# chao1224/pytorch_distributed_nn

Measured on AMD Instinct MI355X. Metric: samples/sec (whole node) ResNet-50 DDP, higher is better.
Workload: dtype bf16; 1 GPU; model=resnet50 (ImageNet layout, 224x224, 1000 classes), global_batch=256, per_gpu_batch=256, image_size=224, parallelism=dp1, optimizer=fused SGD momentum=0.9 wd=5e-5, hipgraph=False, opt_overlap=False

## Files before the change

csrc/kernels/conv3x3.hip:

```cpp
#include "conv_direct.h"

namespace {
using namespace pg;

typedef __attribute__((ext_vector_type(8))) int c3v8i;
typedef __attribute__((ext_vector_type(4))) int c3v4i;
constexpr int C3_AMAX_PARTS = 1024;
#ifndef C3_PRE_J
#define C3_PRE_J 3
#endif
#ifndef C3_F8_PRE_J
#define C3_F8_PRE_J 2
#endif

template <int FMT>
__device__ __forceinline__ uint4 c3_to_fp8(const float* v) {
    constexpr float MX = FMT ? 57344.f : 448.f;
    int w[4];
#pragma unroll
    for (int d = 0; d < 4; ++d) {
        const float c0 = fminf(fmaxf(v[4 * d], -MX), MX), c1 = fminf(fmaxf(v[4 * d + 1], -MX), MX);
        const float c2 = fminf(fmaxf(v[4 * d + 2], -MX), MX), c3 = fminf(fmaxf(v[4 * d + 3], -MX), MX);
        int x = 0;
        if constexpr (FMT) {
// ... 362 lines not shown
        for (int i = 0; i < 4; ++i)
#pragma unroll
            for (int j = 0; j < FN; ++j) acc[i][j] = f32x4_t{0.f, 0.f, 0.f, 0.f};
#pragma unroll
        for (int tap = 0; tap < 9; ++tap) {
            const int dr = tap / 3 - 1, ds = tap % 3 - 1;
            int hp[4];
#pragma unroll
            for (int f = 0; f < 4; ++f) {
                const bool v = pv[f] && (unsigned)(py[f] + dr) < (unsigned)a.H && (unsigned)(px[f] + ds) < (unsigned)a.W;
                hp[f] = v ? hb[f] + dr * a.W + ds : zpx;
            }
            const bf16_t* B = wres + tap * 4096;
#pragma unroll
            for (int ks = 0; ks < 2; ++ks) {
                bf16x8_t af[4], bfr[FN];
                const int q = ks * 4 + (lane >> 4);
#pragma unroll
                for (int f = 0; f < 4; ++f)
                    af[f] = __builtin_bit_cast(bf16x8_t, *reinterpret_cast<const u16x8_t*>(halo + halo_off(hp[f], q)));
#pragma unroll
                for (int f = 0; f < FN; ++f) bfr[f] = frag_kmajor(B, f * 16 + (lane & 15), ks, lane);
#pragma unroll
                for (int fm = 0; fm < 4; ++fm)
#pragma unroll
                    for (int fn = 0; fn < FN; ++fn)
                        acc[fm][fn] = __builtin_amdgcn_mfma_f32_16x16x32_bf16(bfr[fn], af[fm], acc[fm][fn], 0, 0, 0);
            }
        }
        c3_epilogue<NB, EPI>(a, acc, tile, p0, 0, wave, lane, pv);
    }
}

template <int KC, int NB, int EPI, bool PRE, bool FP = false>
__global__ void __launch_bounds__(256, 2) conv1x1_areg_kernel(C3Args a) {
    constexpr int FN = NB / 16, NKS = 2 * KC, K = 64 * KC;
    constexpr int BPT = NB * KC * 8 / 256;
    static_assert(BPT >= 1 && NB * KC * 8 % 256 == 0, "weight step must cover the block");
    extern __shared__ __attribute__((aligned(16))) char smem[];
    bf16_t* const bbuf = reinterpret_cast<bf16_t*>(smem);
    const int tid = threadIdx.x, lane = tid & 63, wave = tid >> 6;
    const int groups = a.ntiles;
    const int t = xcd_remap(blockIdx.x, a.tiles * groups);
    const int tile = t / groups, grp = t - tile * groups;
    const int steps = (a.N / NB) / groups;
    const int c00 = grp * steps;
    const int p0 = tile * C3_BM;

    u16x8_t rb[BPT];
    auto load_b = [&](int s) {
        const int n0 = (c00 + s) * NB;
#pragma unroll
        for (int i = 0; i < BPT; ++i) {
            const int li = tid + 256 * i, row = li / (KC * 8), rem = li - row * (KC * 8);
            rb[i] = *reinterpret_cast<const u16x8_t*>(a.w + (long)(n0 + row) * K + rem * 8);
        }
    };
    auto store_b = [&](int buf) {
        bf16_t* B = bbuf + buf * (KC * NB * 64);
#pragma unroll
        for (int i = 0; i < BPT; ++i) {
            const int li = tid + 256 * i, row = li / (KC * 8), rem = li - row * (KC * 8);
            *reinterpret_cast<u16x8_t*>(B + (rem >> 3) * (NB * 64) + kimg_off(row, rem & 7)) = rb[i];
        }
    };
    load_b(0);

    bool pv[4];
    long prow[4];
#pragma unroll
    for (int fm = 0; fm < 4; ++fm) {
        const int p = p0 + wave * 64 + fm * 16 + (lane & 15);
        pv[fm] = p < a.P;
        prow[fm] = (long)(pv[fm] ? p : a.P - 1) * K;
    }
    bf16x8_t af[NKS][4];
    if constexpr (!PRE) {
        [[maybe_unused]] float* coef = reinterpret_cast<float*>(bbuf + 2 * KC * NB * 64);
        if constexpr (FP) {
            for (int c = tid; c < K; c += 256) {
                coef[c] = a.pro_sc[c];
                coef[K + c] = a.pro_sh[c];
            }
            __syncthreads();
        }
#pragma unroll
        for (int ks = 0; ks < NKS; ++ks)
#pragma unroll
            for (int fm = 0; fm < 4; ++fm) {
                u16x8_t v = *reinterpret_cast<const u16x8_t*>(a.x + prow[fm] + ks * 32 + (lane >> 4) * 8);
                if constexpr (FP) v = fpro_apply_lds<K>(coef, ks * 32 + (lane >> 4) * 8, v);
                af[ks][fm] = __builtin_bit_cast(bf16x8_t, v);
            }
    } else {
        float* coef = reinterpret_cast<float*>(bbuf + 2 * KC * NB * 64);
        {
            const float invL = (float)(1.0 / (double)a.P);
            for (int c = tid; c < K; c += 256) {
                const float is = a.pre_invstd[c], kk = (a.pre_gamma ? a.pre_gamma[c] : 1.f) * is;
                const float dg = a.pre_dgamma[c] * invL, db = a.pre_dbeta[c] * invL;
                coef[c] = kk;
                coef[K + c] = -kk * is * dg;
                coef[2 * K + c] = kk * (a.pre_mean[c] * is * dg - db);
            }
        }
        __syncthreads();
        constexpr int GB = KC == 4 ? 2 : (KC == 2 ? 4 : 2);
#pragma unroll
        for (int g0 = 0; g0 < NKS; g0 += GB) {
            u16x8_t v[GB][4], tv[GB][4];
#pragma unroll
            for (int kk = 0; kk < GB; ++kk)
#pragma unroll
                for (int fm = 0; fm < 4; ++fm) {
                    const long off = prow[fm] + (g0 + kk) * 32 + (lane >> 4) * 8;
                    v[kk][fm] = *reinterpret_cast<const u16x8_t*>(a.x + off);
                    tv[kk][fm] = *reinterpret_cast<const u16x8_t*>(a.pre_t + off);
                }
#pragma unroll
            for (int kk = 0; kk < GB; ++kk) {
                const int k = (g0 + kk) * 32 + (lane >> 4) * 8;
                PreCoef pc;
#pragma unroll
                for (int j = 0; j < 8; ++j) {
                    pc.k[j] = coef[k + j];
                    pc.A[j] = coef[K + k + j];
                    pc.B[j] = coef[2 * K + k + j];
                }
#pragma unroll
                for (int fm = 0; fm < 4; ++fm) {
                    const u16x8_t d = pre_apply(pc, v[kk][fm], tv[kk][fm]);
                    if (a.pre_out && grp == 0 && pv[fm]) *reinterpret_cast<u16x8_t*>(a.pre_out + prow[fm] + k) = d;
                    af[g0 + kk][fm] = __builtin_bit_cast(bf16x8_t, d);
                }
            }
        }
    }
    store_b(0);
    __syncthreads();

    for (int s = 0; s < steps; ++s) {
        const bool more = s + 1 < steps;
        if (more) load_b(s + 1);
        const bf16_t* B = bbuf + (s & 1) * (KC * NB * 64);
        f32x4_t acc[4][FN];
#pragma unroll
        for (int i = 0; i < 4; ++i)
#pragma unroll
            for (int j = 0; j < FN; ++j) acc[i][j] = f32x4_t{0.f, 0.f, 0.f, 0.f};
        bf16x8_t bcur[FN], bnxt[FN];
#pragma unroll
        for (int f = 0; f < FN; ++f) bcur[f] = frag_kmajor(B, f * 16 + (lane & 15), 0, lane);
#pragma unroll
        for (int ks = 0; ks < NKS; ++ks) {
            if (ks + 1 < NKS) {
#pragma unroll
                for (int f = 0; f < FN; ++f)
                    bnxt[f] = frag_kmajor(B + ((ks + 1) >> 1) * (NB * 64), f * 16 + (lane & 15), (ks + 1) & 1, lane);
            }
#pragma unroll
            for (int fm = 0; fm < 4; ++fm)
#pragma unroll
                for (int fn = 0; fn < FN; ++fn)
                    acc[fm][fn] = __builtin_amdgcn_mfma_f32_16x16x32_bf16(bcur[fn], af[ks][fm], acc[fm][fn], 0, 0, 0);
            __builtin_amdgcn_sched_barrier(0);
#pragma unroll
            for (int f = 0; f < FN; ++f) bcur[f] = bnxt[f];
        }
        if (more) store_b((s + 1) & 1);
        c3_epilogue<NB, EPI>(a, acc, tile, p0, (c00 + s) * NB, wave, lane, pv);
        if (more) __syncthreads();
    }
}

int c3r_smem(int W);

__global__ void __launch_bounds__(256) conv3x3_flip_kernel(const bf16_t* __restrict__ w, bf16_t* __restrict__ wt,
                                                           int K, int C) {
    const long n = 9L * K * C;
    for (long i = (long)blockIdx.x * 256 + threadIdx.x; i < n; i += (long)gridDim.x * 256) {
        const int c = (int)(i % C);
        const long r1 = i / C;
        const int tap = (int)(r1 % 9);
        const int k = (int)(r1 / 9);
        wt[((long)c * 9 + (8 - tap)) * K + k] = w[i];
    }
}

int c3_halo_max(int W) {
    const int rows = (C3_BM - 1 + W - 1) / W + 1 + 2;
    return rows * W;
}

__global__ void __launch_bounds__(256) conv3x3_flip8_kernel(const uint8_t* __restrict__ w, uint8_t* __restrict__ wt,
                                                            int K, int C) {
    const long n = 9L * K * C;
    for (long i = (long)blockIdx.x * 256 + threadIdx.x; i < n; i += (long)gridDim.x * 256) {
        const int k = (int)(i % K);
        const long r0 = i / K;
        const int tap = (int)(r0 % 9), c = (int)(r0 / 9);
        wt[i] = w[((long)k * 9 + (8 - tap)) * C + c];
    }
}
// ... 13 lines not shown
    }
    const int grid = a.tiles < grid_cus() ? a.tiles : grid_cus();
    hipLaunchKernelGGL((conv3x3_w64_kernel<EPI>), dim3(grid), dim3(256), sm, st, a);
    PDNN_LAUNCH_RET;
}

template <int NB, int EPI, bool PRE, int F8 = 0, bool FP = false>
int c3_launch(const C3Args& a, hipStream_t st) {
    static int attr_done = 0;
    const int sm = c3_smem<NB>(a.W);
    if (sm > attr_done) {
        (void)hipFuncSetAttribute((const void*)conv3x3_kernel<NB, EPI, PRE, F8, FP>,
                                  hipFuncAttributeMaxDynamicSharedMemorySize, sm);
        attr_done = sm;
    }
    hipLaunchKernelGGL((conv3x3_kernel<NB, EPI, PRE, F8, FP>), dim3(a.tiles * a.ntiles), dim3(256), sm, st, a);
    PDNN_LAUNCH_RET;
}

template <int NB, bool PRE>
int c3_dispatch(const C3Args& a, int epi, hipStream_t st) {
    switch (epi) {
        case C3_BNB: return c3_launch<NB, C3_BNB, PRE>(a, st);
        case C3_STATS: return c3_launch<NB, C3_STATS, PRE>(a, st);
        case C3_RES: return c3_launch<NB, C3_RES, PRE>(a, st);
        default: return c3_launch<NB, C3_PLAIN, PRE>(a, st);
    }
}

}



template <int KC, int NB, int EPI, bool PRE, bool FP = false>
int areg_launch(const C3Args& a, hipStream_t st) {
    constexpr int sm = 2 * KC * NB * 128 + (PRE ? 3 * 64 * KC * 4 : (FP ? 2 * 64 * KC * 4 : 0));
    hipLaunchKernelGGL((conv1x1_areg_kernel<KC, NB, EPI, PRE, FP>), dim3(a.tiles * a.ntiles), dim3(256), sm, st, a);
    PDNN_LAUNCH_RET;
}

template <int KC, int NB, bool PRE>
int areg_dispatch(const C3Args& a, int epi, hipStream_t st) {
    if constexpr (!PRE) {
        if (a.pro_sc) {
            if (epi == C3_STATS) return areg_launch<KC, NB, C3_STATS, false, true>(a, st);
            if (epi == C3_PLAIN) return areg_launch<KC, NB, C3_PLAIN, false, true>(a, st);
            return (int)hipErrorInvalidValue;
        }
    }
    switch (epi) {
        case C3_BNB: return areg_launch<KC, NB, C3_BNB, PRE>(a, st);
        case C3_STATS: return areg_launch<KC, NB, C3_STATS, PRE>(a, st);
        case C3_RES: return areg_launch<KC, NB, C3_RES, PRE>(a, st);
        default: return areg_launch<KC, NB, C3_PLAIN, PRE>(a, st);
    }
}

template <bool PRE>
int areg_run(C3Args& a, int K, int epi, hipStream_t st) {
    const int nb = K == 256 ? 32 : 64;
    const int chunks = a.N / nb;
    int g = 1;
    while (g < chunks && (long)a.tiles * g < 512 && chunks % (2 * g) == 0) g *= 2;
    a.ntiles = g;
    if (K == 64) return areg_dispatch<1, 64, PRE>(a, epi, st);
    if (K == 128) return areg_dispatch<2, 64, PRE>(a, epi, st);
    return areg_dispatch<4, 32, PRE>(a, epi, st);
}

static bool set_pre(C3Args& a, const bf16_t* t, const float* mean, const float* invstd, const float* gamma,
             const float* dgamma, const float* dbeta, bf16_t* out) {
    a.pre_t = t; a.pre_mean = mean; a.pre_invstd = invstd; a.pre_gamma = gamma;
    a.pre_dgamma = dgamma; a.pre_dbeta = dbeta; a.pre_out = out;
    if (!t) return !out;
    return mean && invstd && dgamma && dbeta;
}
static int c3_force() { return pg::tune().conv3x3_force; }

static FastDiv make_fdiv_c3(uint32_t d) {
    FastDiv f;
    f.d = d ? d : 1;
    uint32_t l = 0;
    while ((1ull << l) < f.d) ++l;
    f.s = l;
    f.m = (uint32_t)((((1ull << l) - f.d) << 32) / f.d + 1);
    return f;
}

PDNN_API int pdnn_conv3x3_supported(int Nimg, int H, int W, int C, int N) {
    if (C % 64 || N % 64 || C < 64 || N < 64 || W < 1 || H < 1) return 0;
    if (W < 12 && !c3_force()) return 0;
    if ((long)Nimg * H * W >= (1L << 31) / 2) return 0;
    const int nb = N % 128 == 0 ? 128 : 64;
    const int sm = nb == 128 ? c3_smem<128>(W) : c3_smem<64>(W);
    return sm <= 80 * 1024 ? 1 : 0;
}

PDNN_API int pdnn_conv3x3_force(int f) {
    const int old = c3_force();
    pg::tune().conv3x3_force = f ? 1 : 0;
// ... 84 lines not shown
    C3Args a{};
    a.x = x; a.w = reinterpret_cast<const bf16_t*>(wq); a.y = y;
    a.Nimg = Nimg; a.H = H; a.W = W; a.C = C; a.N = N; a.P = Nimg * H * W;
    a.dW = make_fdiv_c3(W); a.dH = make_fdiv_c3(H);
    a.tiles = (int)cdiv(a.P, C3_BM);
    a.halo_max = c3_halo_max(W);
    a.stats = stats;
    if (!set_pre(a, pre_t, pre_mean, pre_invstd, pre_gamma, pre_dgamma, pre_dbeta, pre_out))
        return (int)hipErrorInvalidValue;
    a.ep_x = bn_x; a.ep_mean = bn_mean; a.ep_invstd = bn_invstd; a.ep_mscale = bn_mscale; a.ep_mshift = bn_mshift;
    if (bn_x && !stats) return (int)hipErrorInvalidValue;
    a.f8_scale = scale; a.f8_inv = inv; a.f8_winv = winv; a.f8_amax = amax;
    a.ntiles = N / 128;
    const bool pre = pre_t != nullptr;
    if (e5m2) {
        if (bn_x) return pre ? c3_launch<128, C3_BNB, true, 2>(a, st) : c3_launch<128, C3_BNB, false, 2>(a, st);
        if (stats) return (int)hipErrorInvalidValue;
        return pre ? c3_launch<128, C3_PLAIN, true, 2>(a, st) : c3_launch<128, C3_PLAIN, false, 2>(a, st);
    }
    if (pre || bn_x) return (int)hipErrorInvalidValue;
    if (!pro_sc != !pro_sh) return (int)hipErrorInvalidValue;
    if (pro_sc) {
        a.pro_sc = pro_sc; a.pro_sh = pro_sh;
        return stats ? c3_launch<128, C3_STATS, false, 1, true>(a, st) : c3_launch<128, C3_PLAIN, false, 1, true>(a, st);
    }
    return stats ? c3_launch<128, C3_STATS, false, 1>(a, st) : c3_launch<128, C3_PLAIN, false, 1>(a, st);
}

PDNN_API int pdnn_conv1x1_panel_supported(long P, int K, int N) {
    const bool k_ok = K == 64 || K == 128 || K == 256;
    return k_ok && N % 64 == 0 && N >= 64 && P > 0 && P < (1L << 30) ? 1 : 0;
}

PDNN_API int pdnn_conv1x1_panel(const bf16_t* x, const bf16_t* w, bf16_t* y, long P, int K, int N, float* stats,
                                const bf16_t* res, const uint8_t* res_mask, const bf16_t* bn_x, const float* bn_mean,
                                const float* bn_invstd, const float* bn_mscale, const float* bn_mshift,
                                const bf16_t* pre_t, const float* pre_mean, const float* pre_invstd,
                                const float* pre_gamma, const float* pre_dgamma, const float* pre_dbeta,
                                bf16_t* pre_out, const float* pro_sc, const float* pro_sh, hipStream_t st) {
    if (!pdnn_conv1x1_panel_supported(P, K, N) || (bn_x && !stats) || (res_mask && !res) || (!pro_sc != !pro_sh) ||
        (pro_sc && (pre_t || bn_x || res)))
        return (int)hipErrorInvalidValue;
    C3Args a{};
    a.x = x; a.w = w; a.y = y; a.C = K; a.N = N; a.P = (int)P;
    a.tiles = (int)cdiv(P, C3_BM);
    a.stats = stats; a.res = res; a.rmask = res_mask;
    a.ep_x = bn_x; a.ep_mean = bn_mean; a.ep_invstd = bn_invstd; a.ep_mscale = bn_mscale; a.ep_mshift = bn_mshift;
    if (!set_pre(a, pre_t, pre_mean, pre_invstd, pre_gamma, pre_dgamma, pre_dbeta, pre_out))
        return (int)hipErrorInvalidValue;
    a.pro_sc = pro_sc; a.pro_sh = pro_sh;
    const int epi = bn_x ? C3_BNB : (stats ? C3_STATS : (res ? C3_RES : C3_PLAIN));
    return pre_t ? areg_run<true>(a, K, epi, st) : areg_run<false>(a, K, epi, st);
}

PDNN_API int pdnn_conv1x1_panel_stats_rows(long P) { return (int)cdiv(P, C3_BM) * 4; }
```

csrc/kernels/conv_direct.h:

```cpp
#pragma once
#include "gemm_common.h"
#include "tuning.h"

namespace {
using namespace pg;

constexpr int C3_BM = 256;
enum { C3_PLAIN = 0, C3_STATS = 1, C3_BNB = 2, C3_RES = 3 };

struct C3Args {
    const bf16_t* x;
    const bf16_t* w;
    bf16_t* y;
    int Nimg, H, W, C, N, P;
    FastDiv dW, dH;
    int tiles, ntiles;
    int halo_max;
    float* stats;
    const bf16_t* res;
    const uint8_t* rmask;
    const bf16_t* ep_x;
    const float *ep_mean, *ep_invstd, *ep_mscale, *ep_mshift;
    const bf16_t* pre_t;
    const float *pre_mean, *pre_invstd, *pre_gamma, *pre_dgamma, *pre_dbeta;
// ... 59 lines not shown
        coef[c] = a.pro_sc[c0 + c];
        coef[CH + c] = a.pro_sh[c0 + c];
    }
}
template <int CH>
__device__ __forceinline__ u16x8_t fpro_apply_lds(const float* coef, int c, const u16x8_t& v) {
    float x[8], sc[8], sh[8];
    unpack8(v, x);
    *reinterpret_cast<float4*>(sc) = *reinterpret_cast<const float4*>(coef + c);
    *reinterpret_cast<float4*>(sc + 4) = *reinterpret_cast<const float4*>(coef + c + 4);
    *reinterpret_cast<float4*>(sh) = *reinterpret_cast<const float4*>(coef + CH + c);
    *reinterpret_cast<float4*>(sh + 4) = *reinterpret_cast<const float4*>(coef + CH + c + 4);
#pragma unroll
    for (int j = 0; j < 8; ++j) x[j] = fmaxf(fmaf(x[j], sc[j], sh[j]), 0.f);
    return pack8(x);
}

__device__ __forceinline__ u16x8_t mask16(const u16x8_t& v, bool ok) {
    const uint32_t m = ok ? 0xFFFFFFFFu : 0u;
    uint4 u = __builtin_bit_cast(uint4, v);
    u.x &= m; u.y &= m; u.z &= m; u.w &= m;
    return __builtin_bit_cast(u16x8_t, u);
}

__device__ __forceinline__ u16x8_t c3_zero8() {
    u16x8_t z = {0, 0, 0, 0, 0, 0, 0, 0};
    return z;
}

__device__ __forceinline__ int halo_off(int hp, int q) {
    return hp * 64 + ((q ^ ((hp >> 1) & 7)) << 3);
}

template <int NB, int EPI>
struct C3PairOps {
    static constexpr bool RES = EPI == C3_RES, BNB = EPI == C3_BNB;
    u16x4_t tv[(RES || BNB) ? 2 : 1][4];
    uint32_t mw[RES ? 4 : 1];
};

template <int NB, int EPI>
__device__ __forceinline__ void c3_load_pair(const C3Args& a, const long (&lrow)[4], int n0, int lg, int fp,
                                             C3PairOps<NB, EPI>& o) {
    constexpr bool RES = EPI == C3_RES, BNB = EPI == C3_BNB;
    if constexpr (RES) {
#pragma unroll
        for (int fm = 0; fm < 4; ++fm)
            o.mw[fm] = a.rmask ? *reinterpret_cast<const uint32_t*>(a.rmask + ((lrow[fm] + n0 + 32 * fp) >> 3))
                               : 0xFFFFFFFFu;
    }
    if constexpr (RES || BNB) {
        const bf16_t* src = BNB ? a.ep_x : a.res;
#pragma unroll
        for (int h = 0; h < 2; ++h) {
            const int n = n0 + (2 * fp + h) * 16 + 4 * lg;
#pragma unroll
            for (int fm = 0; fm < 4; ++fm) o.tv[h][fm] = *reinterpret_cast<const u16x4_t*>(src + lrow[fm] + n);
        }
    }
}

template <int NB, int EPI>
__device__ __forceinline__ void c3_epilogue_rows(const C3Args& a, f32x4_t (&acc)[4][NB / 16], int tile,
                                                 const long (&orow)[4], int n0, int wave, int lane,
                                                 const bool (&pv)[4]) {
    constexpr int FN = NB / 16, NP = FN / 2;
    constexpr bool RES = EPI == C3_RES;
    const int lg = lane >> 4;
    long lrow[4];
#pragma unroll
    for (int fm = 0; fm < 4; ++fm) lrow[fm] = pv[fm] ? orow[fm] : 0;
    C3PairOps<NB, EPI> cur, nxt;
    if constexpr (NP > 1) c3_load_pair<NB, EPI>(a, lrow, n0, lg, 0, cur);
    else if constexpr (RES) {
#pragma unroll
        for (int fm = 0; fm < 4; ++fm)
            cur.mw[fm] = a.rmask ? *reinterpret_cast<const uint32_t*>(a.rmask + ((lrow[fm] + n0) >> 3)) : 0xFFFFFFFFu;
    }
#pragma unroll
    for (int fp = 0; fp < NP; ++fp) {
        if (fp + 1 < NP) c3_load_pair<NB, EPI>(a, lrow, n0, lg, fp + 1, nxt);
        uint32_t pk[4][2][2];
#pragma unroll
        for (int h = 0; h < 2; ++h) {
            const int fn = 2 * fp + h;
            const int n = n0 + fn * 16 + 4 * lg;
            float s[4] = {0, 0, 0, 0}, q[4] = {0, 0, 0, 0};
            float bms[4], bmh[4];
            if constexpr (NP == 1 && (RES || EPI == C3_BNB)) {
                const bf16_t* src = EPI == C3_BNB ? a.ep_x : a.res;
#pragma unroll
                for (int fm = 0; fm < 4; ++fm)
                    cur.tv[h][fm] = pv[fm] ? *reinterpret_cast<const u16x4_t*>(src + orow[fm] + n) : u16x4_t{0, 0, 0, 0};
            }
            if constexpr (EPI == C3_BNB) {
                const float4 m4 = *reinterpret_cast<const float4*>(a.ep_mscale + n);
                const float4 h4 = *reinterpret_cast<const float4*>(a.ep_mshift + n);
                bms[0] = m4.x; bms[1] = m4.y; bms[2] = m4.z; bms[3] = m4.w;
                bmh[0] = h4.x; bmh[1] = h4.y; bmh[2] = h4.z; bmh[3] = h4.w;
            }
#pragma unroll
            for (int fm = 0; fm < 4; ++fm) {
                const bool ok = pv[fm];
                float v[4];
#pragma unroll
                for (int j = 0; j < 4; ++j) v[j] = acc[fm][fn][j];
                if constexpr (RES) {
                    const uint32_t mb = cur.mw[fm] >> (16 * h + 4 * lg);
#pragma unroll
                    for (int j = 0; j < 4; ++j) v[j] += ((mb >> j) & 1) ? bf2f(cur.tv[h][fm][j]) : 0.f;
                }
                if constexpr (EPI == C3_BNB) {
#pragma unroll
                    for (int j = 0; j < 4; ++j) {
                        const float tt = bf2f(cur.tv[h][fm][j]);
                        const float gm = (ok && fmaf(tt, bms[j], bmh[j]) > 0.f) ? bf2f(f2bf(v[j])) : 0.f;
                        v[j] = gm;
                        s[j] += gm;
                        q[j] += gm * tt;
                    }
                } else if constexpr (EPI == C3_STATS) {
                    if (ok) {
#pragma unroll
                        for (int j = 0; j < 4; ++j) {
                            const float r = bf2f(f2bf(v[j]));
                            s[j] += r;
                            q[j] += r * r;
                        }
                    }
                }
                pk[fm][h][0] = pk2bf(v[0], v[1]);
                pk[fm][h][1] = pk2bf(v[2], v[3]);
            }
            if constexpr (EPI == C3_STATS || EPI == C3_BNB) {
#pragma unroll
                for (int j = 0; j < 4; ++j) {
                    s[j] = row16_sum(s[j]);
                    q[j] = row16_sum(q[j]);
                }
                {
                    float* ps = stat_row(a.stats, (long)tile * 4 + wave, a.N) + n;
                    if constexpr (EPI == C3_BNB) {
                        const int j = lane & 3;
                        if ((lane & 12) == 4) {
                            const float qj = (sel4(q, j) - a.ep_mean[n + j] * sel4(s, j)) * a.ep_invstd[n + j];
                            q[0] = q[1] = q[2] = q[3] = qj;
                        }
                    }
                    stat_add_frag(ps, ps + a.N, lane, s, q, true);
                }
            }
        }
#pragma unroll
        for (int fm = 0; fm < 4; ++fm) {
            const auto s0 = __builtin_amdgcn_permlane16_swap(pk[fm][0][0], pk[fm][1][0], false, false);
            const auto s1 = __builtin_amdgcn_permlane16_swap(pk[fm][0][1], pk[fm][1][1], false, false);
            const int n = n0 + (2 * fp + (lg & 1)) * 16 + 8 * (lg >> 1);
            if (pv[fm]) *reinterpret_cast<uint4*>(a.y + orow[fm] + n) = make_uint4(s0[0], s1[0], s0[1], s1[1]);
        }
        if (fp + 1 < NP) cur = nxt;
    }
}

template <int NB, int EPI>
__device__ __forceinline__ void c3_epilogue(const C3Args& a, f32x4_t (&acc)[4][NB / 16], int tile, int p0, int n0,
                                            int wave, int lane, const bool (&pv)[4]) {
    long orow[4];
#pragma unroll
    for (int fm = 0; fm < 4; ++fm) orow[fm] = (long)(p0 + wave * 64 + fm * 16 + (lane & 15)) * a.N;
    c3_epilogue_rows<NB, EPI>(a, acc, tile, orow, n0, wave, lane, pv);
}

}
```

pytorch_distributed_nn_amd/ops/_backend.py:

```python
from __future__ import annotations

import ctypes
import functools
import os
from pathlib import Path

import torch

_LIBDIR = Path(__file__).resolve().parent.parent / "_lib"
_LIB = None
_ERR = None

P = ctypes.c_void_p
I = ctypes.c_int
L = ctypes.c_long
F = ctypes.c_float
D = ctypes.c_double

_SIGS = {
    "pdnn_gemm_nt": [P, L, P, L, P, L, I, I, I, F, P, I, I, P],
    "pdnn_gemm_nn": [P, L, P, L, P, L, I, I, I, F, I, P],
    "pdnn_gemm_tn_acc": [P, L, P, L, P, L, I, I, I, F, P],
    "pdnn_conv_fwd": [P, P, P, I, I, I, I, I, I, I, I, I, I, I, P, P, P, P],
    "pdnn_conv_dgrad": [P, P, P, I, I, I, I, I, I, I, I, I, I, I, P, P, P, P, P, P, P, P, P],
    "pdnn_conv_dgrad_stats_rows": [I, I, I, I, I, I, I],
    "pdnn_conv_wgrad": [P, P, P, I, I, I, I, I, I, I, I, I, I, I, P, P, P],
    "pdnn_gemm_stats_rows": [I],
    "pdnn_conv3x3": [P, P, P, I, I, I, I, I, P, P, P, P, P, P, P, P, I, P, P, P, P, P, P, P, P, P, P],
    "pdnn_conv3x3_supported": [I, I, I, I, I],
    "pdnn_conv3x3s2": [P, P, P, I, I, I, I, I, I, P] + [P] * 5 + [P] * 7 + [P, P, I, P],
    "pdnn_conv3x3s2_supported": [I, I, I, I, I],
    "pdnn_conv3x3s2_wgrad": [P, P, P, I, I, I, I, I, P, P, P, P],
    "pdnn_conv3x3s2_wgrad_supported": [I, I, I, I, I],
    "pdnn_conv3x3s2_wgrad_ws": [I, I, I, I, I],
    "pdnn_conv3x3_fp8_supported": [I, I, I, I, I],
    "pdnn_conv3x3_stats_rows": [I, I, I],
    "pdnn_conv3x3_flip": [P, P, I, I, P],
    "pdnn_conv3x3_flip8": [P, P, I, I, P],
    "pdnn_conv3x3_fp8": [P, P, P, I, I, I, I, I, P] + [P] * 5 + [P] * 7 + [P] * 4 + [I, P, P, P],
    "pdnn_conv3x3_wgrad": [P, P, P, I, I, I, I, I, P, P, P, P],
    "pdnn_conv3x3_wgrad_fp8": [P, P, P, I, I, I, I, I, P, P, P, P, P, P, P, P],
    "pdnn_conv3x3_wgrad_supported": [I, I, I, I, I],
    "pdnn_conv3x3_wgrad_ws": [I, I, I, I, I],
    "pdnn_conv3x3_force": [I],
    "pdnn_tune_set": [ctypes.c_char_p, I],
    "pdnn_tune_get": [ctypes.c_char_p],
    "pdnn_tune_list": [ctypes.c_char_p, I],
    "pdnn_tune_error": [],
    "pdnn_tune_unknown": [],
    "pdnn_set_comm_world": [I],
    "pdnn_grid_cus": [],
    "pdnn_conv1x1_panel": [P, P, P, L, I, I, P, P, P, P, P, P, P, P, P, P, P, P, P, P, P, P, P, P],
    "pdnn_conv1x1_panel_supported": [L, I, I],
    "pdnn_conv1x1_panel_stats_rows": [L],
    "pdnn_conv1x1_wide": [P, P, P, L, I, I] + [P] * 16,
    "pdnn_conv1x1_wide_supported": [L, I, I],
    "pdnn_stem_conv": [P, P, P, I, I, I, I, I, P, P],
    "pdnn_stem_stats_rows": [L],
    "pdnn_stem_conv_nchw": [P, P, P, I, I, I, I, I, P, P],
    "pdnn_stem_wgrad_nchw": [P, P, P, I, I, I, I, I, P, P, P, P, P, P, P, P, P, P, P],
    "pdnn_stem_wgrad_ws": [I, I, I],
    "pdnn_bn_relu_maxpool": [P, P, P, P, P, I, I, I, I, I, I, P],
    "pdnn_set_glds_mode": [I],
    "pdnn_set_pp_mode": [I],
    "pdnn_set_pp_bn": [I],
    "pdnn_set_pp_trace": [P],
    "pdnn_pp_wgrad": [P, L, P, L, P, L, I, I, I, F, P, I, P, I, P],
    "pdnn_pp_wgrad_plan": [I, I, I, I],
    "pdnn_pp_wgrad_splits": [I, I, I],
    "pdnn_pp_wgrad_ws": [I, I, I],
    "pdnn_pp_wgrad_splits_long": [I, I, I],
    "pdnn_pp_gemm_nt_splitk": [P, L, P, L, P, L, I, I, I, P, I, P],
    "pdnn_pp_splitk_splits": [I, I, I],
    "pdnn_transpose_bf16": [P, L, P, L, I, I, P],
    "pdnn_subsample": [P, P, I, I, I, I, I, P],
    "pdnn_transpose_bf16_multi": [P, P, P, P, I, P],
    "pdnn_set_staged_store": [I],
    "pdnn_bn_reduce_rows": [L, I],
    "pdnn_bn_finalize": [P, I, I, D, F, F, P, P, P, P, P, P, P, P, P],
    "pdnn_bn_eval_coeff": [I, F, P, P, P, P, P, P, P],
    "pdnn_bn_stats": [P, L, I, P, P],
    "pdnn_bn_apply": [P, L, I, P, P, P, P, P, I, P, P, P],
    "pdnn_bn_bwd_reduce": [P, P, L, I, P, P, I, P, P, P, P, P, P, P, P, P],
    "pdnn_bn_bwd_finalize": [P, I, I, P, P, I, P, P, P],
    "pdnn_bn_bwd_apply": [P, P, L, I, P, P, P, P, P, I, P, P, P, P, P, P, P, P, P, P, P, P, P],
# ... 176 lines not shown
```

pytorch_distributed_nn_amd/ops/kernels.py:

```python
from __future__ import annotations

import ctypes

import torch

from ._backend import _CUR_DEV, HipError, call, lib, ptr, stream

BF16 = torch.bfloat16
F32 = torch.float32


def _chk(cond, msg):
    if not cond:
        raise ValueError(msg)


def _is_krsc(w):
    K, C, R, S = w.shape
    return w.stride() == (R * S * C, 1, S * C, C)


def _bf16_c(t, name):
    _chk(t.dtype == BF16 and t.is_cuda, f"{name}: expected CUDA bf16, got {t.dtype} {t.device}")
    _chk(t.is_contiguous(), f"{name}: expected contiguous tensor")
# ... 236 lines not shown

def _panel_ok(P, K, N, R, S, st, pad, fwd=False):
    return (_P1["mode"] and R == 1 and S == 1 and st == 1 and pad == 0
            and (lib().pdnn_conv1x1_panel_supported(P, K, N) == 1 or _wide_ok(P, K, N, fwd)))


def _pre_args(pre, x):
    if pre is None:
        return (None,) * 7
    t, mean, inv, gamma, dg, db, dt_out = pre
    _bf16_c(t, "pre.t")
    _chk(t.numel() == x.numel(), "pre: t must have the operand's shape")
    if dt_out is not None:
        _chk(dt_out.numel() == x.numel() and dt_out.dtype == BF16 and dt_out.is_contiguous(), "pre: dt_out")
    return tuple(ptr(v) for v in (t, mean, inv, gamma, dg, db, dt_out))


def conv1x1_panel(x2d, w2d, want_stats=False, res=None, bn=None, res_mask=None, out=None, pre=None, pro=None):
    P, Kc = x2d.shape
    N = w2d.shape[0]
    y = out if out is not None else torch.empty(P, N, device=x2d.device, dtype=BF16)
    slab = None
    t = mean = inv = msc = msh = None
    if want_stats or bn is not None:
        slab = stat_bins(N, x2d.device)
    if bn is not None:
        t, mean, inv, msc, msh = bn
    if Kc >= 512:
        _chk(pro is None, "conv1x1_panel: the forward prologue needs K <= 256")
        call("pdnn_conv1x1_wide", ptr(x2d), ptr(w2d), ptr(y), P, Kc, N, ptr(slab), ptr(res), ptr(res_mask), ptr(t),
             ptr(mean), ptr(inv), ptr(msc), ptr(msh), *_pre_args(pre, x2d), stream())
        return y, slab
    psc, psh = pro if pro is not None else (None, None)
    call("pdnn_conv1x1_panel", ptr(x2d), ptr(w2d), ptr(y), P, Kc, N, ptr(slab), ptr(res), ptr(res_mask), ptr(t),
         ptr(mean), ptr(inv), ptr(msc), ptr(msh), *_pre_args(pre, x2d), ptr(psc), ptr(psh), stream())
    return y, slab


def conv3x3_flip(w):
    K, R, S, C = w.shape
    wt = torch.empty(C, 3, 3, K, device=w.device, dtype=BF16)
    call("pdnn_conv3x3_flip", ptr(w), ptr(wt), K, C, stream())
    return wt


def conv3x3(x, w, want_stats=False, res=None, bn=None, out=None, res_mask=None, pre=None, pro=None):
    Nimg, H, W, C = x.shape
    Ko = w.shape[0]
    y = out if out is not None else torch.empty(Nimg, H, W, Ko, device=x.device, dtype=BF16)
    slab = None
    t = mean = inv = msc = msh = None
    if want_stats or bn is not None:
        slab = stat_bins(Ko, x.device)
    if bn is not None:
        t, mean, inv, msc, msh = bn
    psc, psh = pro if pro is not None else (None, None)
    call("pdnn_conv3x3", ptr(x), ptr(w), ptr(y), Nimg, H, W, C, Ko, ptr(slab), ptr(res), ptr(res_mask), ptr(t),
         ptr(mean), ptr(inv), ptr(msc), ptr(msh), _C3["nb"], *_pre_args(pre, x), ptr(psc), ptr(psh), stream())
    return y, slab


def conv_fwd(x, w, st, pad, pro=None, want_stats=False):
    _bf16_c(x, "conv_fwd.x")
    N, H, W, C = x.shape
    _bf16_c(w, "conv_fwd.w")
    K, R, S, C2 = w.shape
# ... 910 lines not shown
```

pytorch_distributed_nn_amd/tuning.py:

```python
from __future__ import annotations

import os

DEFAULTS = {"side_wgrad": 1, "wide1x1_dgrad": 1, "a2_fold": 1, "wt_prefetch": 0, "wt_layer_batch": 1, "colsum_atomic": 1, "bias_in_wgrad": 1, "s2_halo": 3, "ds_sub": 1, "wgrad1x1_pp_pix": 200704, "gpt2_side_wgrad": 1, "xent_fused": 1, "wgrad_plan_cus": 128}

_VALUES = dict(DEFAULTS)


def _parse(s: str) -> dict:
    out = {}
    for item in filter(None, (p.strip() for p in s.split(","))):
        if "=" not in item:
            raise ValueError(f"PDNN_TUNE: {item!r} is not key=value")
        k, v = item.split("=", 1)
        out[k.strip()] = int(v)
    return out


for _k, _v in _parse(os.environ.get("PDNN_TUNE", "")).items():
    if _k in _VALUES:
        _VALUES[_k] = _v


def get(key: str) -> int:
    return _VALUES[key]


def set(key: str, value: int) -> int:
    if key not in _VALUES:
        raise KeyError(f"unknown tuning key {key!r} (kernel-side keys: ops.kernels.tune_set)")
    old = _VALUES[key]
    _VALUES[key] = int(value)
    return old
```

Measured before the change: 12300 samples/s.

## Add half-height row tiles with higher occupancy for 1x1 panel conv kernel

Templates the 1x1 register-A panel conv kernel and its epilogue on the number of 16-row fragments per wave (4 or 2). The 2-fragment variant uses 128-row pixel tiles and a launch bound of 3 blocks per SM, and the column-group split now targets 768 slots. A heuristic picks the half tile by default for large pixel counts (P >= 50176) in the supported K=128/256 epilogue combinations, and a new tuning key can force either size. The aim is more resident waves and better latency hiding on the big ResNet 1x1 layers. In exchange each block reuses each weight step across fewer rows, weight traffic per output rises, and the register budget per thread is tighter.

```diff
diff --git a/csrc/kernels/conv3x3.hip b/csrc/kernels/conv3x3.hip
--- a/csrc/kernels/conv3x3.hip
+++ b/csrc/kernels/conv3x3.hip
@@ -418,9 +418,11 @@
     }
 }
 
-template <int KC, int NB, int EPI, bool PRE, bool FP = false>
-__global__ void __launch_bounds__(256, 2) conv1x1_areg_kernel(C3Args a) {
+template <int KC, int NB, int EPI, bool PRE, bool FP = false, int FM = 4, int WPS = 2>
+__global__ void __launch_bounds__(256, WPS) conv1x1_areg_kernel(C3Args a) {
     constexpr int FN = NB / 16, NKS = 2 * KC, K = 64 * KC;
+    constexpr int BMA = 64 * FM;
+    static_assert(FM == 4 || FM == 2, "row fragments per wave");
     constexpr int BPT = NB * KC * 8 / 256;
     static_assert(BPT >= 1 && NB * KC * 8 % 256 == 0, "weight step must cover the block");
     extern __shared__ __attribute__((aligned(16))) char smem[];
@@ -431,7 +433,7 @@
     const int tile = t / groups, grp = t - tile * groups;
     const int steps = (a.N / NB) / groups;
     const int c00 = grp * steps;
-    const int p0 = tile * C3_BM;
+    const int p0 = tile * BMA;
 
     u16x8_t rb[BPT];
     auto load_b = [&](int s) {
@@ -452,15 +454,15 @@
     };
     load_b(0);
 
-    bool pv[4];
-    long prow[4];
-#pragma unroll
-    for (int fm = 0; fm < 4; ++fm) {
-        const int p = p0 + wave * 64 + fm * 16 + (lane & 15);
+    bool pv[FM];
+    long prow[FM];
+#pragma unroll
+    for (int fm = 0; fm < FM; ++fm) {
+        const int p = p0 + wave * (16 * FM) + fm * 16 + (lane & 15);
         pv[fm] = p < a.P;
         prow[fm] = (long)(pv[fm] ? p : a.P - 1) * K;
     }
-    bf16x8_t af[NKS][4];
+    bf16x8_t af[NKS][FM];
     if constexpr (!PRE) {
         [[maybe_unused]] float* coef = reinterpret_cast<float*>(bbuf + 2 * KC * NB * 64);
         if constexpr (FP) {
@@ -473,7 +475,7 @@
 #pragma unroll
         for (int ks = 0; ks < NKS; ++ks)
 #pragma unroll
-            for (int fm = 0; fm < 4; ++fm) {
+            for (int fm = 0; fm < FM; ++fm) {
                 u16x8_t v = *reinterpret_cast<const u16x8_t*>(a.x + prow[fm] + ks * 32 + (lane >> 4) * 8);
                 if constexpr (FP) v = fpro_apply_lds<K>(coef, ks * 32 + (lane >> 4) * 8, v);
                 af[ks][fm] = __builtin_bit_cast(bf16x8_t, v);
@@ -491,14 +493,15 @@
             }
         }
         __syncthreads();
-        constexpr int GB = KC == 4 ? 2 : (KC == 2 ? 4 : 2);
+        constexpr int GB4 = KC == 4 ? 2 : (KC == 2 ? 4 : 2);
+        constexpr int GB = GB4 * (4 / FM) < NKS ? GB4 * (4 / FM) : NKS;
 #pragma unroll
         for (int g0 = 0; g0 < NKS; g0 += GB) {
-            u16x8_t v[GB][4], tv[GB][4];
+            u16x8_t v[GB][FM], tv[GB][FM];
 #pragma unroll
             for (int kk = 0; kk < GB; ++kk)
 #pragma unroll
-                for (int fm = 0; fm < 4; ++fm) {
+                for (int fm = 0; fm < FM; ++fm) {
                     const long off = prow[fm] + (g0 + kk) * 32 + (lane >> 4) * 8;
                     v[kk][fm] = *reinterpret_cast<const u16x8_t*>(a.x + off);
                     tv[kk][fm] = *reinterpret_cast<const u16x8_t*>(a.pre_t + off);
@@ -514,7 +517,7 @@
                     pc.B[j] = coef[2 * K + k + j];
                 }
 #pragma unroll
-                for (int fm = 0; fm < 4; ++fm) {
+                for (int fm = 0; fm < FM; ++fm) {
                     const u16x8_t d = pre_apply(pc, v[kk][fm], tv[kk][fm]);
                     if (a.pre_out && grp == 0 && pv[fm]) *reinterpret_cast<u16x8_t*>(a.pre_out + prow[fm] + k) = d;
                     af[g0 + kk][fm] = __builtin_bit_cast(bf16x8_t, d);
@@ -529,9 +532,9 @@
         const bool more = s + 1 < steps;
         if (more) load_b(s + 1);
         const bf16_t* B = bbuf + (s & 1) * (KC * NB * 64);
-        f32x4_t acc[4][FN];
-#pragma unroll
-        for (int i = 0; i < 4; ++i)
+        f32x4_t acc[FM][FN];
+#pragma unroll
+        for (int i = 0; i < FM; ++i)
 #pragma unroll
             for (int j = 0; j < FN; ++j) acc[i][j] = f32x4_t{0.f, 0.f, 0.f, 0.f};
         bf16x8_t bcur[FN], bnxt[FN];
@@ -545,7 +548,7 @@
                     bnxt[f] = frag_kmajor(B + ((ks + 1) >> 1) * (NB * 64), f * 16 + (lane & 15), (ks + 1) & 1, lane);
             }
 #pragma unroll
-            for (int fm = 0; fm < 4; ++fm)
+            for (int fm = 0; fm < FM; ++fm)
 #pragma unroll
                 for (int fn = 0; fn < FN; ++fn)
                     acc[fm][fn] = __builtin_amdgcn_mfma_f32_16x16x32_bf16(bcur[fn], af[ks][fm], acc[fm][fn], 0, 0, 0);
@@ -554,7 +557,7 @@
             for (int f = 0; f < FN; ++f) bcur[f] = bnxt[f];
         }
         if (more) store_b((s + 1) & 1);
-        c3_epilogue<NB, EPI>(a, acc, tile, p0, (c00 + s) * NB, wave, lane, pv);
+        c3_epilogue<NB, EPI, FM>(a, acc, tile, p0, (c00 + s) * NB, wave, lane, pv);
         if (more) __syncthreads();
     }
 }
@@ -634,40 +637,66 @@
 
 
 
-template <int KC, int NB, int EPI, bool PRE, bool FP = false>
+template <int FM>
+constexpr int areg_wps() {
+    return FM == 4 ? 2 : 3;
+}
+
+constexpr bool areg_half_has(int KC, int epi, bool pre, bool fp) {
+    return !fp && (KC == 4 ? epi != C3_STATS : (KC == 2 && epi == C3_RES && pre));
+}
+
+template <int KC, int NB, int EPI, bool PRE, bool FP = false, int FM = 4>
 int areg_launch(const C3Args& a, hipStream_t st) {
-    constexpr int sm = 2 * KC * NB * 128 + (PRE ? 3 * 64 * KC * 4 : (FP ? 2 * 64 * KC * 4 : 0));
-    hipLaunchKernelGGL((conv1x1_areg_kernel<KC, NB, EPI, PRE, FP>), dim3(a.tiles * a.ntiles), dim3(256), sm, st, a);
-    PDNN_LAUNCH_RET;
-}
-
-template <int KC, int NB, bool PRE>
+    if constexpr (FM == 2 && !areg_half_has(KC, EPI, PRE, FP)) {
+        return (int)hipErrorInvalidValue;
+    } else {
+        constexpr int sm = 2 * KC * NB * 128 + (PRE ? 3 * 64 * KC * 4 : (FP ? 2 * 64 * KC * 4 : 0));
+        hipLaunchKernelGGL((conv1x1_areg_kernel<KC, NB, EPI, PRE, FP, FM, areg_wps<FM>()>), dim3(a.tiles * a.ntiles),
+                           dim3(256), sm, st, a);
+        PDNN_LAUNCH_RET;
+    }
+}
+
+template <int KC, int NB, bool PRE, int FM>
 int areg_dispatch(const C3Args& a, int epi, hipStream_t st) {
     if constexpr (!PRE) {
         if (a.pro_sc) {
-            if (epi == C3_STATS) return areg_launch<KC, NB, C3_STATS, false, true>(a, st);
-            if (epi == C3_PLAIN) return areg_launch<KC, NB, C3_PLAIN, false, true>(a, st);
+            if (epi == C3_STATS) return areg_launch<KC, NB, C3_STATS, false, true, FM>(a, st);
+            if (epi == C3_PLAIN) return areg_launch<KC, NB, C3_PLAIN, false, true, FM>(a, st);
             return (int)hipErrorInvalidValue;
         }
     }
     switch (epi) {
-        case C3_BNB: return areg_launch<KC, NB, C3_BNB, PRE>(a, st);
-        case C3_STATS: return areg_launch<KC, NB, C3_STATS, PRE>(a, st);
-        case C3_RES: return areg_launch<KC, NB, C3_RES, PRE>(a, st);
-        default: return areg_launch<KC, NB, C3_PLAIN, PRE>(a, st);
-    }
+        case C3_BNB: return areg_launch<KC, NB, C3_BNB, PRE, false, FM>(a, st);
+        case C3_STATS: return areg_launch<KC, NB, C3_STATS, PRE, false, FM>(a, st);
+        case C3_RES: return areg_launch<KC, NB, C3_RES, PRE, false, FM>(a, st);
+        default: return areg_launch<KC, NB, C3_PLAIN, PRE, false, FM>(a, st);
+    }
+}
+
+static int areg_fm(long P, int K, int epi, bool pre, bool fp, int rows) {
+    if (rows == 4 || !areg_half_has(K / 64, epi, pre, fp)) return 4;
+    return rows == 2 || P >= 50176 ? 2 : 4;
 }
 
 template <bool PRE>
-int areg_run(C3Args& a, int K, int epi, hipStream_t st) {
+int areg_run(C3Args& a, int K, int epi, int rows, hipStream_t st) {
+    const int fm = areg_fm(a.P, K, epi, PRE, a.pro_sc != nullptr, rows);
+    a.tiles = (int)cdiv((long)a.P, 64 * fm);
     const int nb = K == 256 ? 32 : 64;
     const int chunks = a.N / nb;
+    const long slots = fm == 4 ? 512 : 768;
     int g = 1;
-    while (g < chunks && (long)a.tiles * g < 512 && chunks % (2 * g) == 0) g *= 2;
+    while (g < chunks && (long)a.tiles * g < slots && chunks % (2 * g) == 0) g *= 2;
     a.ntiles = g;
-    if (K == 64) return areg_dispatch<1, 64, PRE>(a, epi, st);
-    if (K == 128) return areg_dispatch<2, 64, PRE>(a, epi, st);
-    return areg_dispatch<4, 32, PRE>(a, epi, st);
+    if (fm == 2) {
+        if (K == 128) return areg_dispatch<2, 64, PRE, 2>(a, epi, st);
+        return areg_dispatch<4, 32, PRE, 2>(a, epi, st);
+    }
+    if (K == 64) return areg_dispatch<1, 64, PRE, 4>(a, epi, st);
+    if (K == 128) return areg_dispatch<2, 64, PRE, 4>(a, epi, st);
+    return areg_dispatch<4, 32, PRE, 4>(a, epi, st);
 }
 
 static bool set_pre(C3Args& a, const bf16_t* t, const float* mean, const float* invstd, const float* gamma,
@@ -818,25 +847,36 @@
     return k_ok && N % 64 == 0 && N >= 64 && P > 0 && P < (1L << 30) ? 1 : 0;
 }
 
+PDNN_API int pdnn_conv1x1_panel_tile(const bf16_t* x, const bf16_t* w, bf16_t* y, long P, int K, int N, float* stats,
+                                     const bf16_t* res, const uint8_t* res_mask, const bf16_t* bn_x,
+                                     const float* bn_mean, const float* bn_invstd, const float* bn_mscale,
+                                     const float* bn_mshift, const bf16_t* pre_t, const float* pre_mean,
+                                     const float* pre_invstd, const float* pre_gamma, const float* pre_dgamma,
+                                     const float* pre_dbeta, bf16_t* pre_out, const float* pro_sc, const float* pro_sh,
+                                     int rows, hipStream_t st) {
+    if (!pdnn_conv1x1_panel_supported(P, K, N) || (bn_x && !stats) || (res_mask && !res) || (!pro_sc != !pro_sh) ||
+        (pro_sc && (pre_t || bn_x || res)) || (rows != 0 && rows != 2 && rows != 4))
+        return (int)hipErrorInvalidValue;
+    C3Args a{};
+    a.x = x; a.w = w; a.y = y; a.C = K; a.N = N; a.P = (int)P;
+    a.stats = stats; a.res = res; a.rmask = res_mask;
+    a.ep_x = bn_x; a.ep_mean = bn_mean; a.ep_invstd = bn_invstd; a.ep_mscale = bn_mscale; a.ep_mshift = bn_mshift;
+    if (!set_pre(a, pre_t, pre_mean, pre_invstd, pre_gamma, pre_dgamma, pre_dbeta, pre_out))
+        return (int)hipErrorInvalidValue;
+    a.pro_sc = pro_sc; a.pro_sh = pro_sh;
+    const int epi = bn_x ? C3_BNB : (stats ? C3_STATS : (res ? C3_RES : C3_PLAIN));
+    return pre_t ? areg_run<true>(a, K, epi, rows, st) : areg_run<false>(a, K, epi, rows, st);
+}
+
 PDNN_API int pdnn_conv1x1_panel(const bf16_t* x, const bf16_t* w, bf16_t* y, long P, int K, int N, float* stats,
                                 const bf16_t* res, const uint8_t* res_mask, const bf16_t* bn_x, const float* bn_mean,
                                 const float* bn_invstd, const float* bn_mscale, const float* bn_mshift,
                                 const bf16_t* pre_t, const float* pre_mean, const float* pre_invstd,
                                 const float* pre_gamma, const float* pre_dgamma, const float* pre_dbeta,
                                 bf16_t* pre_out, const float* pro_sc, const float* pro_sh, hipStream_t st) {
-    if (!pdnn_conv1x1_panel_supported(P, K, N) || (bn_x && !stats) || (res_mask && !res) || (!pro_sc != !pro_sh) ||
-        (pro_sc && (pre_t || bn_x || res)))
-        return (int)hipErrorInvalidValue;
-    C3Args a{};
-    a.x = x; a.w = w; a.y = y; a.C = K; a.N = N; a.P = (int)P;
-    a.tiles = (int)cdiv(P, C3_BM);
-    a.stats = stats; a.res = res; a.rmask = res_mask;
-    a.ep_x = bn_x; a.ep_mean = bn_mean; a.ep_invstd = bn_invstd; a.ep_mscale = bn_mscale; a.ep_mshift = bn_mshift;
-    if (!set_pre(a, pre_t, pre_mean, pre_invstd, pre_gamma, pre_dgamma, pre_dbeta, pre_out))
-        return (int)hipErrorInvalidValue;
-    a.pro_sc = pro_sc; a.pro_sh = pro_sh;
-    const int epi = bn_x ? C3_BNB : (stats ? C3_STATS : (res ? C3_RES : C3_PLAIN));
-    return pre_t ? areg_run<true>(a, K, epi, st) : areg_run<false>(a, K, epi, st);
+    return pdnn_conv1x1_panel_tile(x, w, y, P, K, N, stats, res, res_mask, bn_x, bn_mean, bn_invstd, bn_mscale,
+                                   bn_mshift, pre_t, pre_mean, pre_invstd, pre_gamma, pre_dgamma, pre_dbeta, pre_out,
+                                   pro_sc, pro_sh, 0, st);
 }
 
 PDNN_API int pdnn_conv1x1_panel_stats_rows(long P) { return (int)cdiv(P, C3_BM) * 4; }
diff --git a/csrc/kernels/conv_direct.h b/csrc/kernels/conv_direct.h
--- a/csrc/kernels/conv_direct.h
+++ b/csrc/kernels/conv_direct.h
@@ -115,20 +115,20 @@
     return hp * 64 + ((q ^ ((hp >> 1) & 7)) << 3);
 }
 
-template <int NB, int EPI>
+template <int NB, int EPI, int FMR = 4>
 struct C3PairOps {
     static constexpr bool RES = EPI == C3_RES, BNB = EPI == C3_BNB;
-    u16x4_t tv[(RES || BNB) ? 2 : 1][4];
-    uint32_t mw[RES ? 4 : 1];
+    u16x4_t tv[(RES || BNB) ? 2 : 1][FMR];
+    uint32_t mw[RES ? FMR : 1];
 };
 
-template <int NB, int EPI>
-__device__ __forceinline__ void c3_load_pair(const C3Args& a, const long (&lrow)[4], int n0, int lg, int fp,
-                                             C3PairOps<NB, EPI>& o) {
+template <int NB, int EPI, int FMR = 4>
+__device__ __forceinline__ void c3_load_pair(const C3Args& a, const long (&lrow)[FMR], int n0, int lg, int fp,
+                                             C3PairOps<NB, EPI, FMR>& o) {
     constexpr bool RES = EPI == C3_RES, BNB = EPI == C3_BNB;
     if constexpr (RES) {
 #pragma unroll
-        for (int fm = 0; fm < 4; ++fm)
+        for (int fm = 0; fm < FMR; ++fm)
             o.mw[fm] = a.rmask ? *reinterpret_cast<const uint32_t*>(a.rmask + ((lrow[fm] + n0 + 32 * fp) >> 3))
                                : 0xFFFFFFFFu;
     }
@@ -138,32 +138,32 @@
         for (int h = 0; h < 2; ++h) {
             const int n = n0 + (2 * fp + h) * 16 + 4 * lg;
 #pragma unroll
-            for (int fm = 0; fm < 4; ++fm) o.tv[h][fm] = *reinterpret_cast<const u16x4_t*>(src + lrow[fm] + n);
+            for (int fm = 0; fm < FMR; ++fm) o.tv[h][fm] = *reinterpret_cast<const u16x4_t*>(src + lrow[fm] + n);
         }
     }
 }
 
-template <int NB, int EPI>
-__device__ __forceinline__ void c3_epilogue_rows(const C3Args& a, f32x4_t (&acc)[4][NB / 16], int tile,
-                                                 const long (&orow)[4], int n0, int wave, int lane,
-                                                 const bool (&pv)[4]) {
+template <int NB, int EPI, int FMR = 4>
+__device__ __forceinline__ void c3_epilogue_rows(const C3Args& a, f32x4_t (&acc)[FMR][NB / 16], int tile,
+                                                 const long (&orow)[FMR], int n0, int wave, int lane,
+                                                 const bool (&pv)[FMR]) {
     constexpr int FN = NB / 16, NP = FN / 2;
     constexpr bool RES = EPI == C3_RES;
     const int lg = lane >> 4;
-    long lrow[4];
-#pragma unroll
-    for (int fm = 0; fm < 4; ++fm) lrow[fm] = pv[fm] ? orow[fm] : 0;
-    C3PairOps<NB, EPI> cur, nxt;
-    if constexpr (NP > 1) c3_load_pair<NB, EPI>(a, lrow, n0, lg, 0, cur);
+    long lrow[FMR];
+#pragma unroll
+    for (int fm = 0; fm < FMR; ++fm) lrow[fm] = pv[fm] ? orow[fm] : 0;
+    C3PairOps<NB, EPI, FMR> cur, nxt;
+    if constexpr (NP > 1) c3_load_pair<NB, EPI, FMR>(a, lrow, n0, lg, 0, cur);
     else if constexpr (RES) {
 #pragma unroll
-        for (int fm = 0; fm < 4; ++fm)
+        for (int fm = 0; fm < FMR; ++fm)
             cur.mw[fm] = a.rmask ? *reinterpret_cast<const uint32_t*>(a.rmask + ((lrow[fm] + n0) >> 3)) : 0xFFFFFFFFu;
     }
 #pragma unroll
     for (int fp = 0; fp < NP; ++fp) {
-        if (fp + 1 < NP) c3_load_pair<NB, EPI>(a, lrow, n0, lg, fp + 1, nxt);
-        uint32_t pk[4][2][2];
+        if (fp + 1 < NP) c3_load_pair<NB, EPI, FMR>(a, lrow, n0, lg, fp + 1, nxt);
+        uint32_t pk[FMR][2][2];
 #pragma unroll
         for (int h = 0; h < 2; ++h) {
             const int fn = 2 * fp + h;
@@ -173,7 +173,7 @@
             if constexpr (NP == 1 && (RES || EPI == C3_BNB)) {
                 const bf16_t* src = EPI == C3_BNB ? a.ep_x : a.res;
 #pragma unroll
-                for (int fm = 0; fm < 4; ++fm)
+                for (int fm = 0; fm < FMR; ++fm)
                     cur.tv[h][fm] = pv[fm] ? *reinterpret_cast<const u16x4_t*>(src + orow[fm] + n) : u16x4_t{0, 0, 0, 0};
             }
             if constexpr (EPI == C3_BNB) {
@@ -183,7 +183,7 @@
                 bmh[0] = h4.x; bmh[1] = h4.y; bmh[2] = h4.z; bmh[3] = h4.w;
             }
 #pragma unroll
-            for (int fm = 0; fm < 4; ++fm) {
+            for (int fm = 0; fm < FMR; ++fm) {
                 const bool ok = pv[fm];
                 float v[4];
 #pragma unroll
@@ -235,7 +235,7 @@
             }
         }
 #pragma unroll
-        for (int fm = 0; fm < 4; ++fm) {
+        for (int fm = 0; fm < FMR; ++fm) {
             const auto s0 = __builtin_amdgcn_permlane16_swap(pk[fm][0][0], pk[fm][1][0], false, false);
             const auto s1 = __builtin_amdgcn_permlane16_swap(pk[fm][0][1], pk[fm][1][1], false, false);
             const int n = n0 + (2 * fp + (lg & 1)) * 16 + 8 * (lg >> 1);
@@ -245,13 +245,13 @@
     }
 }
 
-template <int NB, int EPI>
-__device__ __forceinline__ void c3_epilogue(const C3Args& a, f32x4_t (&acc)[4][NB / 16], int tile, int p0, int n0,
-                                            int wave, int lane, const bool (&pv)[4]) {
-    long orow[4];
-#pragma unroll
-    for (int fm = 0; fm < 4; ++fm) orow[fm] = (long)(p0 + wave * 64 + fm * 16 + (lane & 15)) * a.N;
-    c3_epilogue_rows<NB, EPI>(a, acc, tile, orow, n0, wave, lane, pv);
-}
-
-}
+template <int NB, int EPI, int FMR = 4>
+__device__ __forceinline__ void c3_epilogue(const C3Args& a, f32x4_t (&acc)[FMR][NB / 16], int tile, int p0, int n0,
+                                            int wave, int lane, const bool (&pv)[FMR]) {
+    long orow[FMR];
+#pragma unroll
+    for (int fm = 0; fm < FMR; ++fm) orow[fm] = (long)(p0 + wave * (16 * FMR) + fm * 16 + (lane & 15)) * a.N;
+    c3_epilogue_rows<NB, EPI, FMR>(a, acc, tile, orow, n0, wave, lane, pv);
+}
+
+}
diff --git a/pytorch_distributed_nn_amd/ops/_backend.py b/pytorch_distributed_nn_amd/ops/_backend.py
--- a/pytorch_distributed_nn_amd/ops/_backend.py
+++ b/pytorch_distributed_nn_amd/ops/_backend.py
@@ -51,6 +51,7 @@
     "pdnn_set_comm_world": [I],
     "pdnn_grid_cus": [],
     "pdnn_conv1x1_panel": [P, P, P, L, I, I, P, P, P, P, P, P, P, P, P, P, P, P, P, P, P, P, P, P],
+    "pdnn_conv1x1_panel_tile": [P, P, P, L, I, I, P, P, P, P, P, P, P, P, P, P, P, P, P, P, P, P, P, I, P],
     "pdnn_conv1x1_panel_supported": [L, I, I],
     "pdnn_conv1x1_panel_stats_rows": [L],
     "pdnn_conv1x1_wide": [P, P, P, L, I, I] + [P] * 16,
diff --git a/pytorch_distributed_nn_amd/ops/kernels.py b/pytorch_distributed_nn_amd/ops/kernels.py
--- a/pytorch_distributed_nn_amd/ops/kernels.py
+++ b/pytorch_distributed_nn_amd/ops/kernels.py
@@ -292,6 +292,11 @@
              ptr(mean), ptr(inv), ptr(msc), ptr(msh), *_pre_args(pre, x2d), stream())
         return y, slab
     psc, psh = pro if pro is not None else (None, None)
+    rows = _tuning.get("areg_rows")
+    if rows:
+        call("pdnn_conv1x1_panel_tile", ptr(x2d), ptr(w2d), ptr(y), P, Kc, N, ptr(slab), ptr(res), ptr(res_mask),
+             ptr(t), ptr(mean), ptr(inv), ptr(msc), ptr(msh), *_pre_args(pre, x2d), ptr(psc), ptr(psh), rows, stream())
+        return y, slab
     call("pdnn_conv1x1_panel", ptr(x2d), ptr(w2d), ptr(y), P, Kc, N, ptr(slab), ptr(res), ptr(res_mask), ptr(t),
          ptr(mean), ptr(inv), ptr(msc), ptr(msh), *_pre_args(pre, x2d), ptr(psc), ptr(psh), stream())
     return y, slab
diff --git a/pytorch_distributed_nn_amd/tuning.py b/pytorch_distributed_nn_amd/tuning.py
--- a/pytorch_distributed_nn_amd/tuning.py
+++ b/pytorch_distributed_nn_amd/tuning.py
@@ -2,7 +2,7 @@
 
 import os
 
-DEFAULTS = {"side_wgrad": 1, "wide1x1_dgrad": 1, "a2_fold": 1, "wt_prefetch": 0, "wt_layer_batch": 1, "colsum_atomic": 1, "bias_in_wgrad": 1, "s2_halo": 3, "ds_sub": 1, "wgrad1x1_pp_pix": 200704, "gpt2_side_wgrad": 1, "xent_fused": 1, "wgrad_plan_cus": 128}
+DEFAULTS = {"side_wgrad": 1, "wide1x1_dgrad": 1, "a2_fold": 1, "wt_prefetch": 0, "wt_layer_batch": 1, "colsum_atomic": 1, "bias_in_wgrad": 1, "s2_halo": 3, "ds_sub": 1, "wgrad1x1_pp_pix": 200704, "gpt2_side_wgrad": 1, "xent_fused": 1, "wgrad_plan_cus": 128, "areg_rows": 0}
 
 _VALUES = dict(DEFAULTS)
 
```

After: 12300 samples/s. Within noise of the previous version (-0.0%).
